# Starlight0798/gymRL

Hardware: AMD Instinct MI355X
Metric: env-steps/sec at N envs/GPU (PPO LunarLander), 1/2/4/8 GPUs + %HBM roofline (higher is better)
Workload: dtype f32; 1 GPU; PPO LunarLander-v3, 4096 vectorised envs per MI355X (BASELINE.json configs[1]); envs_per_gpu=4096, rollout_len=2048, num_epochs=10, num_minibatches=32, minibatch=262144, model=ActorCritic 8-256-256-{256-4,256-1} tanh, 200,965 params, parallelism=single GPU

## Files before the change

### gymrl_amd/csrc/env_lunar.hip

```cpp
#include "env_lunar_device.hpp"

using namespace gymrl;
using namespace gymrl::lunar;

namespace {

__global__ __launch_bounds__(kEnvBlock) void lunar_reset_kernel(void* buf, int n, uint64_t seed,
                                                                int64_t env_id0,
                                                                float* __restrict__ obs_out) {
  __shared__ uint32_t lds_words[kLdsWords * kEnvBlock];
  const Lds lds{lds_words + threadIdx.x};
  LunarState st(buf, n);
  const int role = threadIdx.x & 3;
  const int i = blockIdx.x * kEnvsPerBlock + (threadIdx.x >> 2);
  if (i >= n) return;
  World W;
  float fx, fy, rew, o[8]; bool term;
  init_episode(W, lds, seed, (uint64_t)(env_id0 + i), 0u, fx, fy);
  env_step_once(W, lds, role, 0, seed, (uint64_t)(env_id0 + i), 0u, 0u, fx, fy, o, rew, term);
  world_io(W, lds, role, st.words, n, i, true);
  if (role == 0) {
    st.ep.ep_ret[i] = 0.0; st.ep.ep_len[i] = 0; st.ep.episode[i] = 0u;
    st.spare_episode[i] = kNoSpare;
  }
  store_obs_quad(obs_out, i, role, o);
}

__global__ __launch_bounds__(kEnvBlock) void lunar_refill_kernel(void* buf, int n, uint64_t seed,
                                                                 int64_t env_id0) {
  __shared__ uint32_t lds_words[kLdsWords * kEnvBlock];
  const Lds lds{lds_words + threadIdx.x};
  LunarState st(buf, n);
  const int role = threadIdx.x & 3;
  const int i = blockIdx.x * kEnvsPerBlock + (threadIdx.x >> 2);
  if (i >= n) return;
  const uint32_t want = st.ep.episode[i] + 1u;
  lunar_refill_quad(st, lds, n, i, role, st.spare_episode[i] != want, want, seed, env_id0);
}

__global__ __launch_bounds__(kEnvBlock) void lunar_step_kernel(
    void* buf, int n, uint64_t seed, int64_t env_id0, const int32_t* __restrict__ action,
    float* __restrict__ obs_out, float* __restrict__ term_obs_out, float* __restrict__ rew_out,
    uint8_t* __restrict__ terminated_out, uint8_t* __restrict__ truncated_out,
    uint8_t* __restrict__ done_out, float* __restrict__ ep_ret_out,
    int32_t* __restrict__ ep_len_out, double* __restrict__ ep_stats) {
  __shared__ uint32_t lds_words[kLdsWords * kEnvBlock];
  const Lds lds{lds_words + threadIdx.x};
  const LunarState st(buf, n);
  const int role = threadIdx.x & 3;
  const int i = blockIdx.x * kEnvsPerBlock + (threadIdx.x >> 2);
  const bool valid = i < n;
  const StepOut out{obs_out, term_obs_out, rew_out, terminated_out, truncated_out, done_out, ep_ret_out, ep_len_out, ep_stats};
  float o_next[8];
  lunar_step_quad(st, lds, n, i, role, valid, valid ? action[i] : 0, seed, env_id0, out, o_next);
}

inline int cdiv(int a, int b) { return (a + b - 1) / b; }

}

namespace gymrl {

size_t lunar_state_bytes(int n) { return LunarState(nullptr, n).bytes; }

int lunar_reset(void* state, int n, uint64_t seed, int64_t env_id0, float* obs_out, hipStream_t s) {
  hipLaunchKernelGGL(lunar_reset_kernel, dim3(cdiv(n, kEnvsPerBlock)), dim3(kEnvBlock), 0, s, state, n, seed,
                     env_id0, obs_out);
  GYMRL_CHECK_LAUNCH();
  return 0;
}

int lunar_refill(void* state, int n, uint64_t seed, int64_t env_id0, hipStream_t s) {
  hipLaunchKernelGGL(lunar_refill_kernel, dim3(cdiv(n, kEnvsPerBlock)), dim3(kEnvBlock), 0, s, state, n, seed, env_id0);
  GYMRL_CHECK_LAUNCH();
  return 0;
}

int lunar_step(void* state, int n, uint64_t seed, int64_t env_id0, const int32_t* action,
               float* obs_out, float* term_obs_out, float* rew_out, uint8_t* terminated_out,
               uint8_t* truncated_out, uint8_t* done_out, float* ep_ret_out, int32_t* ep_len_out,
               double* ep_stats, hipStream_t s) {
  hipLaunchKernelGGL(lunar_step_kernel, dim3(cdiv(n, kEnvsPerBlock)), dim3(kEnvBlock), 0, s, state, n, seed,
                     env_id0, action, obs_out, term_obs_out, rew_out, terminated_out, truncated_out,
                     done_out, ep_ret_out, ep_len_out, ep_stats);
  GYMRL_CHECK_LAUNCH();
  return 0;
}

}
```

### gymrl_amd/csrc/env_lunar_device.hpp

```cpp
#pragma once
#include "env_common.hpp"

namespace gymrl {
namespace lunar {


constexpr float kScale = 30.0f;
constexpr float kW = 600.0f / kScale;
constexpr float kH = 400.0f / kScale;
constexpr float kHelipadY = kH / 4.0f;
constexpr float kLegDown = 18.0f / kScale;
constexpr float kLegAway = 20.0f / kScale;
constexpr float kDt = 1.0f / 50.0f;
constexpr int kVelIters = 180, kPosIters = 60, kMaxSteps = 1000;
constexpr float kLinearSlopSqMax = 0x1.a36e30p-16f;
constexpr float kLinearSlop = 0.005f, kAngularSlop = 2.0f / 180.0f * 3.14159265359f;
constexpr float kPolyRadius = 2.0f * kLinearSlop;
constexpr float kMaxLinCorr = 0.2f, kMaxAngCorr = 8.0f / 180.0f * 3.14159265359f;
constexpr float kBaumgarte = 0.2f;
constexpr float kMaxTranslation = 2.0f, kMaxRotation = 0.5f * 3.14159265359f;
constexpr float kTimeToSleep = 0.5f, kLinSleepTol = 0.01f, kAngSleepTol = 2.0f / 180.0f * 3.14159265359f;
constexpr float kMotorTorque = 40.0f;

__device__ constexpr float kInvM[3] = {0.20761245674740486f, 14.0625f, 14.0625f};
__device__ constexpr float kInvI[3] = {1.2757043935679302f, 558.3639705882352f, 558.3639705882352f};
constexpr float kHullLcY = 0.10130718954248369f;
__device__ constexpr float kHullVx[6] = {17.f / 30, 17.f / 30, 14.f / 30, -14.f / 30, -17.f / 30, -17.f / 30};
__device__ constexpr float kHullVy[6] = {-10.f / 30, 0.f, 17.f / 30, 17.f / 30, 0.f, -10.f / 30};
__device__ constexpr float kHullNx[6] = {1.0f, 0.9847835588179369f, 0.0f, -0.9847835588179369f, -1.0f, 0.0f};
__device__ constexpr float kHullNy[6] = {0.0f, 0.17378533390904766f, 1.0f, 0.17378533390904766f, 0.0f, -1.0f};
__device__ constexpr float kLegVx[4] = {-2.f / 30, 2.f / 30, 2.f / 30, -2.f / 30};
__device__ constexpr float kLegVy[4] = {-8.f / 30, -8.f / 30, 8.f / 30, 8.f / 30};
__device__ constexpr float kLegNx[4] = {0.0f, 1.0f, 0.0f, -1.0f};
__device__ constexpr float kLegNy[4] = {-1.0f, 0.0f, 1.0f, 0.0f};

typedef float v2f __attribute__((ext_vector_type(2)));
struct Body { float cx, cy, a, vx, vy, w; };

struct Joint {
  float ix, iy, iz, im;
  int state;
};

struct ContactPt { float lpx, lpy; uint32_t key; float ni, ti; };
struct Manifold {
  int count;
  int faceB;
  float lnx, lny, lpx, lpy;
  ContactPt p[2];
};

constexpr int kMfWords = 16;
constexpr int kVcWords = 17;
constexpr int kLdsWords = 2 * kMfWords + 2 * kVcWords;
constexpr int kQuad = 4;
constexpr int kEnvsPerBlock = kEnvBlock / kQuad;

#ifdef GYMRL_LUNAR_PROF
#define LUNAR_PROF_MARK(var) const unsigned long long var = wall_clock64()
#define LUNAR_PROF_ADD(lds, slot, t0, t1) do { if ((lds).prof && (threadIdx.x & 63) == 0) (lds).prof[slot] += (t1) - (t0); } while (0)
#else
#define LUNAR_PROF_MARK(var)
#define LUNAR_PROF_ADD(lds, slot, t0, t1)
#endif

struct Lds {
  uint32_t* w;
#ifdef GYMRL_LUNAR_PROF
  unsigned long long* prof;
#endif
  uint32_t* park = nullptr;
#ifdef GYMRL_LUNAR_PROF
  unsigned long long* envp = nullptr;
  int envn = 0;
#endif
  __device__ __forceinline__ float& mf(int s, int f) const { return reinterpret_cast<float*>(w)[(s * kMfWords + f) * kEnvBlock]; }
  __device__ __forceinline__ uint32_t& mu(int s, int f) const { return w[(s * kMfWords + f) * kEnvBlock]; }
  __device__ __forceinline__ float& vc(int s, int f) const { return reinterpret_cast<float*>(w)[(2 * kMfWords + s * kVcWords + f) * kEnvBlock]; }
  __device__ __forceinline__ uint32_t& vu(int s, int f) const { return w[(2 * kMfWords + s * kVcWords + f) * kEnvBlock]; }
};

template <int R>
__device__ __forceinline__ float quad_bcast(float x) {
  return __int_as_float(__builtin_amdgcn_update_dpp(0, __float_as_int(x), R * 0x55, 0xF, 0xF, true));
}
template <int CTRL>
__device__ __forceinline__ float quad_perm(float x) {
  return __int_as_float(__builtin_amdgcn_update_dpp(0, __float_as_int(x), CTRL, 0xF, 0xF, true));
}
constexpr int kRot1 = 0xC9;
constexpr int kRot2 = 0xD2;
constexpr int kSwap01 = 0xE1;
template <int R>
__device__ __forceinline__ uint32_t quad_bcast_u(uint32_t x) {
  return (uint32_t)__builtin_amdgcn_update_dpp(0, (int)x, R * 0x55, 0xF, 0xF, true);
}
enum { MF_COUNT = 0, MF_FACEB = 1, MF_LNX = 2, MF_LNY = 3, MF_LPX = 4, MF_LPY = 5, MF_P0 = 6, MF_P1 = 11,
       P_LPX = 0, P_LPY = 1, P_KEY = 2, P_NI = 3, P_TI = 4 };
enum { VC_COUNT = 0, VC_NX = 1, VC_NY = 2, VC_RX0 = 3, VC_RY0 = 4, VC_RX1 = 5, VC_RY1 = 6, VC_NM0 = 7, VC_NM1 = 8,
       VC_TM0 = 9, VC_TM1 = 10, VC_K11 = 11, VC_K12 = 12, VC_K22 = 13, VC_I11 = 14, VC_I12 = 15, VC_I22 = 16 };

struct World {
  Body b[3];
  float sleep[3];
  Joint j[2];
  int edge0;
  uint32_t touching;
  float ty[11];
  uint32_t flags;
  float prev_shaping;
};

__device__ __forceinline__ float cross2(float ax, float ay, float bx, float by) { return ax * by - ay * bx; }
__device__ __forceinline__ float dot2(float ax, float ay, float bx, float by) { return ax * bx + ay * by; }
__device__ __forceinline__ float clampf(float x, float lo, float hi) { return fmaxf(lo, fminf(x, hi)); }

__device__ __forceinline__ float leg_sign(int L) { return L == 0 ? -1.0f : 1.0f; }
__device__ __forceinline__ float joint_lower(int L) { return L == 0 ? 0.4f : -0.9f; }
__device__ __forceinline__ float joint_upper(int L) { return L == 0 ? 0.9f : -0.4f; }

template <int NV>
__device__ __forceinline__ void collide_edge_polygon(Manifold& mf, const float* __restrict__ VX,
                                                     const float* __restrict__ VY,
                                                     const float* __restrict__ NX,
                                                     const float* __restrict__ NY, float px, float py,
                                                     float qs, float qc, float ccx, float ccy,
                                                     float v1x, float v1y, float v2x, float v2y) {
  mf.count = 0;
  float wx[NV], wy[NV], wnx[NV], wny[NV];
#pragma unroll
  for (int i = 0; i < NV; ++i) {
    wx[i] = (qc * VX[i] - qs * VY[i]) + px;
    wy[i] = (qs * VX[i] + qc * VY[i]) + py;
    wnx[i] = qc * NX[i] - qs * NY[i];
    wny[i] = qs * NX[i] + qc * NY[i];
  }
  float ex = v2x - v1x, ey = v2y - v1y;
  const float el = sqrtf(ex * ex + ey * ey);
  const float inv = 1.0f / el;
  ex *= inv; ey *= inv;
  const float n1x = ey, n1y = -ex;
  const float offset1 = dot2(n1x, n1y, ccx - v1x, ccy - v1y);
  const bool front = offset1 >= 0.0f;
  const float Nx = front ? n1x : -n1x, Ny = front ? n1y : -n1y;
  const float radius = 2.0f * kPolyRadius;

  float esep = 3.4e38f;
#pragma unroll
  for (int i = 0; i < NV; ++i) {
    const float s = dot2(Nx, Ny, wx[i] - v1x, wy[i] - v1y);
    if (s < esep) esep = s;
  }
  if (esep > radius) return;
  float psep = -3.4e38f;
  int pidx = -1;
  bool separated = false;
#pragma unroll
  for (int i = 0; i < NV; ++i) {
    const float nx = -wnx[i], ny = -wny[i];
    const float s1 = dot2(nx, ny, wx[i] - v1x, wy[i] - v1y);
    const float s2 = dot2(nx, ny, wx[i] - v2x, wy[i] - v2y);
    const float s = fminf(s1, s2);
    if (!separated) {
      if (s > radius) { separated = true; }
      else if (s > psep) { psep = s; pidx = i; }
    }
  }
  if (separated) return;
  const bool use_edge = (pidx < 0) || !(psep > 0.98f * esep + 0.001f);

  float i0x, i0y, i1x, i1y;
  uint32_t id0, id1;
  float rv1x, rv1y, rv2x, rv2y, rnx, rny;
  int ri1, ri2;
  if (use_edge) {
    int best = 0;
    float bestv = dot2(Nx, Ny, wnx[0], wny[0]);
#pragma unroll
    for (int i = 1; i < NV; ++i) {
      const float v = dot2(Nx, Ny, wnx[i], wny[i]);
      if (v < bestv) { bestv = v; best = i; }
    }
    const int b2 = best + 1 < NV ? best + 1 : 0;
    i0x = wx[0]; i0y = wy[0]; i1x = wx[0]; i1y = wy[0];
#pragma unroll
    for (int i = 0; i < NV; ++i) {
      if (i == best) { i0x = wx[i]; i0y = wy[i]; }
      if (i == b2) { i1x = wx[i]; i1y = wy[i]; }
    }
    id0 = 0u | ((uint32_t)best << 8) | (1u << 16) | (0u << 24);
    id1 = 0u | ((uint32_t)b2 << 8) | (1u << 16) | (0u << 24);
    if (front) { ri1 = 0; ri2 = 1; rv1x = v1x; rv1y = v1y; rv2x = v2x; rv2y = v2y; rnx = n1x; rny = n1y; }
    else { ri1 = 1; ri2 = 0; rv1x = v2x; rv1y = v2y; rv2x = v1x; rv2y = v1y; rnx = -n1x; rny = -n1y; }
  } else {
    i0x = v1x; i0y = v1y; i1x = v2x; i1y = v2y;
    id0 = 0u | ((uint32_t)pidx << 8) | (0u << 16) | (1u << 24);
    id1 = 0u | ((uint32_t)pidx << 8) | (0u << 16) | (1u << 24);
    ri1 = pidx; ri2 = pidx + 1 < NV ? pidx + 1 : 0;
    rv1x = wx[0]; rv1y = wy[0]; rv2x = wx[0]; rv2y = wy[0]; rnx = wnx[0]; rny = wny[0];
#pragma unroll
    for (int i = 0; i < NV; ++i) {
      if (i == ri1) { rv1x = wx[i]; rv1y = wy[i]; rnx = wnx[i]; rny = wny[i]; }
      if (i == ri2) { rv2x = wx[i]; rv2y = wy[i]; }
    }
  }
  const float sn1x = rny, sn1y = -rnx;
  const float so1 = dot2(sn1x, sn1y, rv1x, rv1y);
  const float so2 = dot2(-sn1x, -sn1y, rv2x, rv2y);

  float c0x, c0y, c1x, c1y; uint32_t cid0, cid1; int np = 0;
  {
    const float d0 = dot2(sn1x, sn1y, i0x, i0y) - so1;
    const float d1 = dot2(sn1x, sn1y, i1x, i1y) - so1;
    c0x = c0y = c1x = c1y = 0.0f; cid0 = cid1 = 0u;
    if (d0 <= 0.0f) { c0x = i0x; c0y = i0y; cid0 = id0; np = 1; }
    if (d1 <= 0.0f) { if (np == 0) { c0x = i1x; c0y = i1y; cid0 = id1; } else { c1x = i1x; c1y = i1y; cid1 = id1; } ++np; }
    if (d0 * d1 < 0.0f) {
      const float t = d0 / (d0 - d1);
      const float nxp = i0x + t * (i1x - i0x), nyp = i0y + t * (i1y - i0y);
      const uint32_t nid = (uint32_t)ri1 | (((id0 >> 8) & 0xFFu) << 8) | (0u << 16) | (1u << 24);
      if (np == 0) { c0x = nxp; c0y = nyp; cid0 = nid; } else { c1x = nxp; c1y = nyp; cid1 = nid; }
      ++np;
    }
  }
  if (np < 2) return;
  float e0x, e0y, e1x, e1y; uint32_t eid0, eid1; np = 0;
  {
    const float d0 = dot2(-sn1x, -sn1y, c0x, c0y) - so2;
    const float d1 = dot2(-sn1x, -sn1y, c1x, c1y) - so2;
    e0x = e0y = e1x = e1y = 0.0f; eid0 = eid1 = 0u;
    if (d0 <= 0.0f) { e0x = c0x; e0y = c0y; eid0 = cid0; np = 1; }
    if (d1 <= 0.0f) { if (np == 0) { e0x = c1x; e0y = c1y; eid0 = cid1; } else { e1x = c1x; e1y = c1y; eid1 = cid1; } ++np; }
    if (d0 * d1 < 0.0f) {
      const float t = d0 / (d0 - d1);
      const float nxp = c0x + t * (c1x - c0x), nyp = c0y + t * (c1y - c0y);
      const uint32_t nid = (uint32_t)ri2 | (((cid0 >> 8) & 0xFFu) << 8) | (0u << 16) | (1u << 24);
      if (np == 0) { e0x = nxp; e0y = nyp; eid0 = nid; } else { e1x = nxp; e1y = nyp; eid1 = nid; }
      ++np;
    }
  }
  if (np < 2) return;

  mf.faceB = use_edge ? 0 : 1;
  if (use_edge) { mf.lnx = rnx; mf.lny = rny; mf.lpx = rv1x; mf.lpy = rv1y; }
  else {
    mf.lnx = NX[0]; mf.lny = NY[0]; mf.lpx = VX[0]; mf.lpy = VY[0];
#pragma unroll
    for (int i = 0; i < NV; ++i) if (i == ri1) { mf.lnx = NX[i]; mf.lny = NY[i]; mf.lpx = VX[i]; mf.lpy = VY[i]; }
  }
  int cnt = 0;
#pragma unroll
  for (int k = 0; k < 2; ++k) {
    const float qx = k == 0 ? e0x : e1x, qy = k == 0 ? e0y : e1y;
    const uint32_t qid = k == 0 ? eid0 : eid1;
    const float sep = dot2(rnx, rny, qx - rv1x, qy - rv1y);
    if (sep <= radius) {
      float lx, ly; uint32_t key;
      if (use_edge) {
        const float dx = qx - px, dy = qy - py;
        lx = qc * dx + qs * dy; ly = -qs * dx + qc * dy;
        key = qid;
      } else {
        lx = qx; ly = qy;
        key = ((qid >> 8) & 0xFFu) | ((qid & 0xFFu) << 8) | (((qid >> 24) & 0xFFu) << 16) | (((qid >> 16) & 0xFFu) << 24);
// ... 270 lines not shown
    }
    quad_share_velocity(B, me);
  }

  float jrAx[2], jrAy[2], jrBx[2], jrBy[2];
  float K11[2], K12[2], K13[2], K22[2], K23[2], K33[2], mmass[2];
  {
    float qsA, qcA;
    det_sincosf(B[0].a, &qsA, &qcA);
#pragma unroll
    for (int jj = 0; jj < 2; ++jj) {
      const int L = 1 - jj;
      const int bi = L + 1;
      float qsB, qcB;
      det_sincosf(B[bi].a, &qsB, &qcB);
      const float lax = 0.0f - 0.0f, lay = 0.0f - kHullLcY;
      const float lbx = leg_sign(L) * kLegAway, lby = kLegDown;
      jrAx[L] = qcA * lax - qsA * lay; jrAy[L] = qsA * lax + qcA * lay;
      jrBx[L] = qcB * lbx - qsB * lby; jrBy[L] = qsB * lbx + qcB * lby;
      const float mA = kInvM[0], mB = kInvM[bi], iA = kInvI[0], iB = kInvI[bi];
      K11[L] = mA + mB + jrAy[L] * jrAy[L] * iA + jrBy[L] * jrBy[L] * iB;
      K12[L] = -jrAy[L] * jrAx[L] * iA - jrBy[L] * jrBx[L] * iB;
      K13[L] = -jrAy[L] * iA - jrBy[L] * iB;
      K22[L] = mA + mB + jrAx[L] * jrAx[L] * iA + jrBx[L] * jrBx[L] * iB;
      K23[L] = jrAx[L] * iA + jrBx[L] * iB;
      K33[L] = iA + iB;
      mmass[L] = 1.0f / (iA + iB);
      Joint& J = W.j[L];
      const float ang = B[bi].a - B[0].a;
      if (ang <= joint_lower(L)) { if (J.state != 1) J.iz = 0.0f; J.state = 1; }
      else if (ang >= joint_upper(L)) { if (J.state != 2) J.iz = 0.0f; J.state = 2; }
      else { J.state = 0; J.iz = 0.0f; }
      const float Px = J.ix, Py = J.iy;
      B[0].vx -= mA * Px; B[0].vy -= mA * Py;
      B[0].w -= iA * (cross2(jrAx[L], jrAy[L], Px, Py) + J.im + J.iz);
      B[bi].vx += mB * Px; B[bi].vy += mB * Py;
      B[bi].w += iB * (cross2(jrBx[L], jrBy[L], Px, Py) + J.im + J.iz);
    }
  }

  LUNAR_PROF_MARK(pt2);
  LUNAR_PROF_ADD(lds, 1, pt1, pt2);
  float jpAx[2], jpAy[2], jpBx[2], jpBy[2];
  float c1x[2], c1y[2], c1z[2], det3i[2], det2i[2], lim_sign[2];
  bool at_limit[2];
#pragma unroll
  for (int L = 0; L < 2; ++L) {
    const float a11 = K11[L], a12 = K12[L], a13 = K13[L], a22 = K22[L], a23 = K23[L], a33 = K33[L];
    c1x[L] = a22 * a33 - a23 * a23; c1y[L] = a23 * a13 - a12 * a33; c1z[L] = a12 * a23 - a22 * a13;
    float det = a11 * c1x[L] + a12 * c1y[L] + a13 * c1z[L];
    if (det != 0.0f) det = 1.0f / det;
    det3i[L] = det;
    float d2 = a11 * a22 - a12 * a12;
    if (d2 != 0.0f) d2 = 1.0f / d2;
    det2i[L] = d2;
    jpAx[L] = -jrAy[L]; jpAy[L] = jrAx[L]; jpBx[L] = -jrBy[L]; jpBy[L] = jrBx[L];
    at_limit[L] = W.j[L].state != 0;
    lim_sign[L] = W.j[L].state == 1 ? 1.0f : -1.0f;
  }
  const bool r0 = role == 0, r1 = role == 1, r2 = role == 2;
  auto lane3 = [&](float x, float y, float z) { return r0 ? x : (r1 ? y : (r2 ? z : 0.0f)); };
  float JPA[2], JPB[2], C1[2], P2[2], Q2[2], A2[2], P3[2], Q3[2], A3[2], A3C[2], D2[2], MBv[2], IBz[2];
#pragma unroll
  for (int L = 0; L < 2; ++L) {
    const float a11 = K11[L], a12 = K12[L], a13 = K13[L], a22 = K22[L], a23 = K23[L], a33 = K33[L];
    JPA[L] = lane3(jpAx[L], jpAy[L], 0.0f); JPB[L] = lane3(jpBx[L], jpBy[L], 0.0f);
    C1[L] = lane3(c1x[L], c1y[L], c1z[L]);
    P2[L] = lane3(a23, a33, a13); Q2[L] = lane3(a13, a23, a33); A2[L] = lane3(a13, a11, a12);
    P3[L] = lane3(a23, a12, a22); Q3[L] = lane3(a12, a22, a23); A3[L] = lane3(a12, a13, a11);
    A3C[L] = lane3(a13, a23, 0.0f); D2[L] = lane3(a22, a11, 0.0f);
    MBv[L] = lane3(kInvM[L + 1], kInvM[L + 1], kInvI[L + 1]); IBz[L] = r2 ? kInvI[L + 1] : 0.0f;
  }
  const float MAv = lane3(kInvM[0], kInvM[0], kInvI[0]), IAz = r2 ? kInvI[0] : 0.0f;
  float VA = lane3(B[0].vx, B[0].vy, B[0].w);
  float VB[2] = {lane3(B[1].vx, B[1].vy, B[1].w), lane3(B[2].vx, B[2].vy, B[2].w)};
  float JI[2] = {lane3(W.j[0].ix, W.j[0].iy, W.j[0].iz), lane3(W.j[1].ix, W.j[1].iy, W.j[1].iz)};
  float IM[2] = {W.j[0].im, W.j[1].im};
  const float maxImp = h * kMotorTorque;
#define SB __builtin_amdgcn_sched_barrier(0)
#define USEL(c, a, b) (__builtin_unpredictable(c) ? (a) : (b))
  float zb[2];
  zb[1] = quad_perm<0xAA>(JI[1]) * A3C[1];
  zb[0] = 0.0f;
  float lim_nan[2] = {at_limit[0] ? lim_sign[0] : __builtin_nanf(""), at_limit[1] ? lim_sign[1] : __builtin_nanf("")};
  asm volatile("" : "+v"(lim_nan[0]), "+v"(lim_nan[1]));
  auto joints = [&]() {
#pragma unroll
    for (int jj = 0; jj < 2; ++jj) {
      const int L = 1 - jj;
      const bool lim = at_limit[L];
      float t = VB[L] - VA; SB;
      t = t - 0.3f * leg_sign(L); SB;
      float imp = -mmass[L] * t; SB;
      float nw = IM[L] + imp; SB;
      nw = __builtin_amdgcn_fmed3f(nw, -maxImp, maxImp); SB;
      imp = nw - IM[L]; IM[L] = nw; SB;
      const float mb_ = IBz[L] * imp; SB;
      VB[L] = VB[L] + mb_; SB;
      const float ma_ = IAz * imp; SB;
      VA = VA - ma_; SB;
      const float xb = quad_perm<0xAA>(VB[L]) * JPB[L]; SB;
      float c = VB[L] + xb; SB;
      const float xa = quad_perm<0xAA>(VA) * JPA[L]; SB;
      c = c - VA; SB;
      c = c - xa; SB;
      const float u1 = c * C1[L]; SB;
      const float zc = zb[L] - c; SB;
      const float q2 = quad_perm<kRot1>(c) * Q2[L]; SB;
      const float q3 = quad_perm<kRot2>(c) * Q3[L]; SB;
      const float m2 = c * P2[L] - q2; SB;
      const float m3 = c * P3[L] - q3; SB;
      float s1 = quad_perm<kRot1>(u1) + u1; SB;
      const float u2 = A2[L] * m2; SB;
      const float u3 = A3[L] * m3; SB;
      s1 = quad_perm<kRot2>(u1) + s1; SB;
      const float rr = USEL(lim, zc, -c); SB;
      float s2 = quad_perm<kRot1>(u2) + u2; SB;
      float s3 = quad_perm<kRot1>(u3) + u3; SB;
      const float d2r = D2[L] * rr; SB;
      s2 = quad_perm<kRot2>(u2) + s2; SB;
      s3 = quad_perm<kRot2>(u3) + s3; SB;
      const float r2_ = quad_perm<kSwap01>(rr) * K12[L]; SB;
      float sel = USEL(r1, s2, s3); SB;
      sel = USEL(r0, s1, sel); SB;
      const float nsol = -(det3i[L] * sel); SB;
      const float newJ = JI[L] + nsol; SB;
      const float uu = d2r - r2_; SB;
      const float u = det2i[L] * uu; SB;
      const float rt = quad_perm<0xAA>(newJ) * lim_nan[L]; SB;
      const float altz = USEL(lim, -JI[L], 0.0f); SB;
      const float alt = USEL(r2, altz, u); SB;
      float ip;
      asm("v_cmp_nge_f32 vcc, %1, 0\n\tv_cndmask_b32_e32 %0, %2, %3, vcc" : "=v"(ip) : "v"(rt), "v"(nsol), "v"(alt) : "vcc"); SB;
      JI[L] = JI[L] + ip; SB;
      zb[1 - L] = quad_perm<0xAA>(JI[1 - L]) * A3C[1 - L]; SB;
      const float ay = quad_perm<0x55>(ip) * jrAx[L]; SB;
      const float ax = quad_perm<0x00>(ip) * jrAy[L]; SB;
      const float by = quad_perm<0x55>(ip) * jrBx[L]; SB;
      const float bx = quad_perm<0x00>(ip) * jrBy[L]; SB;
      const float crA = ay - ax; SB;
      const float crB = by - bx; SB;
      const float wA = crA + ip; SB;
      const float wB = crB + ip; SB;
      float tA = USEL(r2, wA, ip); SB;
      float tB = USEL(r2, wB, ip); SB;
      tA = MAv * tA; SB;
      tB = MBv[L] * tB; SB;
      VA = VA - tA; SB;
      VB[L] = VB[L] + tB; SB;
    }
  };
#undef SB
#undef USEL
  auto contacts = [&]() {
    if (any_contact) {
      Body me;
      me.cx = me.cy = me.a = 0.0f;
      me.vx = sel3(mb, quad_bcast<0>(VA), quad_bcast<0>(VB[0]), quad_bcast<0>(VB[1]));
      me.vy = sel3(mb, quad_bcast<1>(VA), quad_bcast<1>(VB[0]), quad_bcast<1>(VB[1]));
      me.w = sel3(mb, quad_bcast<2>(VA), quad_bcast<2>(VB[0]), quad_bcast<2>(VB[1]));
#pragma unroll
      for (int s = 0; s < 2; ++s) {
        const int vcount = vcn[s];
        if (vcount > 0) {
          const float nx = vcf[s][VC_NX - 1], ny = vcf[s][VC_NY - 1], tx = ny, ty = -nx;
          const float rx0 = vcf[s][VC_RX0 - 1], ry0 = vcf[s][VC_RY0 - 1], rx1 = vcf[s][VC_RX1 - 1], ry1 = vcf[s][VC_RY1 - 1];
          float ni0 = vim[s][0], ti0 = vim[s][1], ni1 = vim[s][2], ti1 = vim[s][3];
          {
            const float dvx = me.vx + (-me.w * ry0), dvy = me.vy + (me.w * rx0);
            const float vt = dot2(dvx, dvy, tx, ty);
            float lam = vcf[s][VC_TM0 - 1] * (-vt);
            const float maxF = fr_ * ni0;
            const float nw = clampf(ti0 + lam, -maxF, maxF);
            lam = nw - ti0; ti0 = nw;
            const float Px = lam * tx, Py = lam * ty;
            me.vx += mB_ * Px; me.vy += mB_ * Py;
            me.w += iB_ * cross2(rx0, ry0, Px, Py);
          }
          if (vcount == 2) {
            const float dvx = me.vx + (-me.w * ry1), dvy = me.vy + (me.w * rx1);
            const float vt = dot2(dvx, dvy, tx, ty);
            float lam = vcf[s][VC_TM1 - 1] * (-vt);
            const float maxF = fr_ * ni1;
            const float nw = clampf(ti1 + lam, -maxF, maxF);
            lam = nw - ti1; ti1 = nw;
            const float Px = lam * tx, Py = lam * ty;
            me.vx += mB_ * Px; me.vy += mB_ * Py;
            me.w += iB_ * cross2(rx1, ry1, Px, Py);
          }
          if (vcount == 1) {
            const float dvx = me.vx + (-me.w * ry0), dvy = me.vy + (me.w * rx0);
            const float vn = dot2(dvx, dvy, nx, ny);
            float lam = -vcf[s][VC_NM0 - 1] * vn;
            const float nw = fmaxf(ni0 + lam, 0.0f);
            lam = nw - ni0; ni0 = nw;
            const float Px = lam * nx, Py = lam * ny;
            me.vx += mB_ * Px; me.vy += mB_ * Py;
            me.w += iB_ * cross2(rx0, ry0, Px, Py);
          } else {
            const float k11 = vcf[s][VC_K11 - 1], k12 = vcf[s][VC_K12 - 1], k22 = vcf[s][VC_K22 - 1];
            const float a1 = ni0, a2 = ni1;
            const float dv1x = me.vx + (-me.w * ry0), dv1y = me.vy + (me.w * rx0);
            const float dv2x = me.vx + (-me.w * ry1), dv2y = me.vy + (me.w * rx1);
            float vn1 = dot2(dv1x, dv1y, nx, ny), vn2 = dot2(dv2x, dv2y, nx, ny);
            const float b1 = vn1 - (k11 * a1 + k12 * a2);
            const float b2 = vn2 - (k12 * a1 + k22 * a2);
            float x1 = -(vcf[s][VC_I11 - 1] * b1 + vcf[s][VC_I12 - 1] * b2);
            float x2 = -(vcf[s][VC_I12 - 1] * b1 + vcf[s][VC_I22 - 1] * b2);
            bool ok = (x1 >= 0.0f && x2 >= 0.0f);
            if (!ok) {
              x1 = -vcf[s][VC_NM0 - 1] * b1; x2 = 0.0f;
              vn2 = k12 * x1 + b2;
              ok = (x1 >= 0.0f && vn2 >= 0.0f);
            }
            if (!ok) {
              x1 = 0.0f; x2 = -vcf[s][VC_NM1 - 1] * b2;
              vn1 = k12 * x2 + b1;
              ok = (x2 >= 0.0f && vn1 >= 0.0f);
            }
            if (!ok) {
              x1 = 0.0f; x2 = 0.0f;
              ok = (b1 >= 0.0f && b2 >= 0.0f);
            }
            if (ok) {
              const float d1 = x1 - a1, d2 = x2 - a2;
              const float P1x = d1 * nx, P1y = d1 * ny, P2x = d2 * nx, P2y = d2 * ny;
              me.vx += mB_ * (P1x + P2x); me.vy += mB_ * (P1y + P2y);
              me.w += iB_ * (cross2(rx0, ry0, P1x, P1y) + cross2(rx1, ry1, P2x, P2y));
              ni0 = x1; ni1 = x2;
            }
          }
          vim[s][0] = ni0; vim[s][1] = ti0;
          if (vcount == 2) { vim[s][2] = ni1; vim[s][3] = ti1; }
        }
      }
      VA = lane3(quad_bcast<0>(me.vx), quad_bcast<0>(me.vy), quad_bcast<0>(me.w));
      VB[0] = lane3(quad_bcast<1>(me.vx), quad_bcast<1>(me.vy), quad_bcast<1>(me.w));
      VB[1] = lane3(quad_bcast<2>(me.vx), quad_bcast<2>(me.vy), quad_bcast<2>(me.w));
    }
  };
  if (__builtin_amdgcn_ballot_w64(any_contact) == 0ull) {
#pragma nounroll
    for (int it = 0; it < kVelIters; ++it) joints();
  } else {
#pragma nounroll
    for (int it = 0; it < kVelIters; ++it) { joints(); contacts(); }
  }
  B[0].vx = quad_bcast<0>(VA); B[0].vy = quad_bcast<1>(VA); B[0].w = quad_bcast<2>(VA);
#pragma unroll
  for (int L = 0; L < 2; ++L) {
    B[L + 1].vx = quad_bcast<0>(VB[L]); B[L + 1].vy = quad_bcast<1>(VB[L]); B[L + 1].w = quad_bcast<2>(VB[L]);
    W.j[L].ix = quad_bcast<0>(JI[L]); W.j[L].iy = quad_bcast<1>(JI[L]); W.j[L].iz = quad_bcast<2>(JI[L]);
    W.j[L].im = quad_bcast<2>(IM[L]);
  }
  LUNAR_PROF_MARK(pt3);
  LUNAR_PROF_ADD(lds, 2, pt2, pt3);
#ifdef GYMRL_LUNAR_PROF
  const bool wave_contact = __builtin_amdgcn_ballot_w64(any_contact) != 0ull;
  LUNAR_PROF_ADD(lds, wave_contact ? 6 : 7, pt2, pt3);
#endif
  if (my_contact) {
#pragma unroll
    for (int s = 0; s < 2; ++s) {
      if (vcn[s] > 0) {
        lds.mf(s, MF_P0 + P_NI) = vim[s][0]; lds.mf(s, MF_P0 + P_TI) = vim[s][1];
        if (vcn[s] == 2) { lds.mf(s, MF_P1 + P_NI) = vim[s][2]; lds.mf(s, MF_P1 + P_TI) = vim[s][3]; }
      }
    }
  }

#pragma unroll
  for (int b = 0; b < 3; ++b) {
    float tx = h * B[b].vx, ty = h * B[b].vy;
    if (dot2(tx, ty, tx, ty) > kMaxTranslation * kMaxTranslation) {
      const float ratio = kMaxTranslation / sqrtf(dot2(tx, ty, tx, ty));
      B[b].vx *= ratio; B[b].vy *= ratio;
    }
    const float rot = h * B[b].w;
    if (rot * rot > kMaxRotation * kMaxRotation) {
      const float ratio = kMaxRotation / fabsf(rot);
      B[b].w *= ratio;
    }
    B[b].cx += h * B[b].vx; B[b].cy += h * B[b].vy; B[b].a += h * B[b].w;
  }

  LUNAR_PROF_MARK(pt4);
  LUNAR_PROF_ADD(lds, 3, pt3, pt4);
#ifdef GYMRL_LUNAR_PROF
  int prof_pos_iters = 0;
#endif
  bool position_solved = false;
  float plim_value[2], plim_slop[2], plim_lo[2], plim_hi[2];
#pragma unroll
  for (int L = 0; L < 2; ++L) {
    const bool lower = W.j[L].state == 1;
    plim_value[L] = lower ? joint_lower(L) : joint_upper(L);
    plim_slop[L] = lower ? kAngularSlop : -kAngularSlop;
    plim_lo[L] = lower ? -kMaxAngCorr : 0.0f;
    plim_hi[L] = lower ? 0.0f : kMaxAngCorr;
  }
  int pcnt[2] = {0, 0};
  bool pfaceB[2] = {false, false};
  float plnx[2], plny[2], plpx[2], plpy[2], pqx[2][2], pqy[2][2];
#pragma unroll
  for (int s = 0; s < 2; ++s) {
    plnx[s] = plny[s] = plpx[s] = plpy[s] = 0.0f;
    pqx[s][0] = pqx[s][1] = pqy[s][0] = pqy[s][1] = 0.0f;
    if (my_contact) {
      pcnt[s] = (int)lds.mu(s, MF_COUNT);
      pfaceB[s] = lds.mu(s, MF_FACEB) != 0u;
      plnx[s] = lds.mf(s, MF_LNX); plny[s] = lds.mf(s, MF_LNY);
      plpx[s] = lds.mf(s, MF_LPX); plpy[s] = lds.mf(s, MF_LPY);
#pragma unroll
      for (int k = 0; k < 2; ++k) {
        pqx[s][k] = lds.mf(s, MF_P0 + 5 * k + P_LPX); pqy[s][k] = lds.mf(s, MF_P0 + 5 * k + P_LPY);
      }
    }
  }
#pragma nounroll
  for (int it = 0; it < kPosIters; ++it) {
    float min_sep = 0.0f;
    if (any_contact) {
      Body me = select_body(B, mb);
      float my_min = 0.0f;
#pragma unroll
      for (int s = 0; s < 2; ++s) {
        const int cnt = pcnt[s];
        if (cnt > 0) {
          const bool faceB = pfaceB[s];
          const float lnx = plnx[s], lny = plny[s], lpx = plpx[s], lpy = plpy[s];
#pragma unroll
          for (int k = 0; k < 2; ++k) {
            if (k < cnt) {
              const float qx = pqx[s][k], qy = pqy[s][k];
              float px, py, qs, qc;
              body_xf(me, lcy_, px, py, qs, qc);
              float nx, ny, ptx, pty, sep;
              if (!faceB) {
                nx = lnx; ny = lny;
                const float clx = (qc * qx - qs * qy) + px, cly = (qs * qx + qc * qy) + py;
                sep = dot2(clx - lpx, cly - lpy, nx, ny) - kPolyRadius - kPolyRadius;
                ptx = clx; pty = cly;
              } else {
                nx = qc * lnx - qs * lny; ny = qs * lnx + qc * lny;
                const float ppx = (qc * lpx - qs * lpy) + px, ppy = (qs * lpx + qc * lpy) + py;
                sep = dot2(qx - ppx, qy - ppy, nx, ny) - kPolyRadius - kPolyRadius;
                ptx = qx; pty = qy;
                nx = -nx; ny = -ny;
              }
              const float rx = ptx - me.cx, ry = pty - me.cy;
              my_min = fminf(my_min, sep);
              const float C = clampf(kBaumgarte * (sep + kLinearSlop), -kMaxLinCorr, 0.0f);
              const float rn = cross2(rx, ry, nx, ny);
              const float K = mB_ + iB_ * rn * rn;
              const float imp = K > 0.0f ? -C / K : 0.0f;
              const float Px = imp * nx, Py = imp * ny;
              me.cx += mB_ * Px; me.cy += mB_ * Py;
              me.a += iB_ * cross2(rx, ry, Px, Py);
            }
          }
        }
      }
      quad_share_position(B, me);
      min_sep = fminf(fminf(quad_bcast<0>(my_min), quad_bcast<1>(my_min)), quad_bcast<2>(my_min));
    }
    const bool contacts_ok = min_sep >= -3.0f * kLinearSlop;
    bool joints_ok = true;
#pragma unroll
    for (int jj = 0; jj < 2; ++jj) {
      const int L = 1 - jj;
      const int bi = L + 1;
      const float mA = kInvM[0], mB = kInvM[bi], iA = kInvI[0], iB = kInvI[bi];
      const bool lim = at_limit[L];
      const float Cang = (B[bi].a - B[0].a) - plim_value[L];
      const float angErr = lim ? -(lim_sign[L] * Cang) : 0.0f;
      const float Cc = clampf(Cang + plim_slop[L], plim_lo[L], plim_hi[L]);
      const float limImp = lim ? -mmass[L] * Cc : 0.0f;
      B[0].a -= iA * limImp; B[bi].a += iB * limImp;
      float qsA, qcA, qsB, qcB;
      {
        float sn, cs;
        det_sincosf((role & 1) ? B[bi].a : B[0].a, &sn, &cs);
        qsA = quad_bcast<0>(sn); qcA = quad_bcast<0>(cs);
        qsB = quad_bcast<1>(sn); qcB = quad_bcast<1>(cs);
      }
      const float lax = 0.0f, lay = 0.0f - kHullLcY;
      const float lbx = leg_sign(L) * kLegAway, lby = kLegDown;
      const float rAx = qcA * lax - qsA * lay, rAy = qsA * lax + qcA * lay;
      const float rBx = qcB * lbx - qsB * lby, rBy = qsB * lbx + qcB * lby;
      const float Cx = B[bi].cx + rBx - B[0].cx - rAx, Cy = B[bi].cy + rBy - B[0].cy - rAy;
      const float posErr2 = Cx * Cx + Cy * Cy;
      const float k11 = mA + mB + iA * rAy * rAy + iB * rBy * rBy;
      const float k12 = -iA * rAx * rAy - iB * rBx * rBy;
      const float k22 = mA + mB + iA * rAx * rAx + iB * rBx * rBx;
      float det = k11 * k22 - k12 * k12;
      if (det != 0.0f) det = 1.0f / det;
      const float impx = -(det * (k22 * Cx - k12 * Cy)), impy = -(det * (k11 * Cy - k12 * Cx));
      B[0].cx -= mA * impx; B[0].cy -= mA * impy;
      B[0].a -= iA * cross2(rAx, rAy, impx, impy);
// ... 357 lines not shown
```

Before: 7.237 million env-steps/s.

## Specialize contact velocity sweep by wave contact shape and use DPP select asm

The contact velocity solver loop is split into three template variants chosen per wave by ballot: general two-point manifolds, one-point with a second slot, and one-point single-slot. This drops the 2x2 block solver and second-slot branches from the 180-iteration inner loop when no lane in the wave needs them. The quad broadcast/select of body velocities is rewritten as inline DPP v_cndmask asm with precomputed role masks to cut instruction count. An env var forces the general path, at the cost of more code size and hand-written asm that depends on the quad role layout.

```diff
diff --git a/gymrl_amd/csrc/env_lunar.hip b/gymrl_amd/csrc/env_lunar.hip
--- a/gymrl_amd/csrc/env_lunar.hip
+++ b/gymrl_amd/csrc/env_lunar.hip
@@ -1,3 +1,5 @@
+#include <cstdlib>
+
 #include "env_lunar_device.hpp"
 
 using namespace gymrl;
@@ -43,9 +45,10 @@
     float* __restrict__ obs_out, float* __restrict__ term_obs_out, float* __restrict__ rew_out,
     uint8_t* __restrict__ terminated_out, uint8_t* __restrict__ truncated_out,
     uint8_t* __restrict__ done_out, float* __restrict__ ep_ret_out,
-    int32_t* __restrict__ ep_len_out, double* __restrict__ ep_stats) {
+    int32_t* __restrict__ ep_len_out, double* __restrict__ ep_stats, int general_sweep) {
   __shared__ uint32_t lds_words[kLdsWords * kEnvBlock];
-  const Lds lds{lds_words + threadIdx.x};
+  Lds lds{lds_words + threadIdx.x};
+  lds.general_sweep = general_sweep != 0;
   const LunarState st(buf, n);
   const int role = threadIdx.x & 3;
   const int i = blockIdx.x * kEnvsPerBlock + (threadIdx.x >> 2);
@@ -80,9 +83,11 @@
                float* obs_out, float* term_obs_out, float* rew_out, uint8_t* terminated_out,
                uint8_t* truncated_out, uint8_t* done_out, float* ep_ret_out, int32_t* ep_len_out,
                double* ep_stats, hipStream_t s) {
+  const char* gs = getenv("GYMRL_LUNAR_GENERAL_SWEEP");
+  const int general_sweep = gs && gs[0] == '1';
   hipLaunchKernelGGL(lunar_step_kernel, dim3(cdiv(n, kEnvsPerBlock)), dim3(kEnvBlock), 0, s, state, n, seed,
                      env_id0, action, obs_out, term_obs_out, rew_out, terminated_out, truncated_out,
-                     done_out, ep_ret_out, ep_len_out, ep_stats);
+                     done_out, ep_ret_out, ep_len_out, ep_stats, general_sweep);
   GYMRL_CHECK_LAUNCH();
   return 0;
 }
diff --git a/gymrl_amd/csrc/env_lunar_device.hpp b/gymrl_amd/csrc/env_lunar_device.hpp
--- a/gymrl_amd/csrc/env_lunar_device.hpp
+++ b/gymrl_amd/csrc/env_lunar_device.hpp
@@ -74,6 +74,7 @@
   unsigned long long* envp = nullptr;
   int envn = 0;
 #endif
+  bool general_sweep = false;
   __device__ __forceinline__ float& mf(int s, int f) const { return reinterpret_cast<float*>(w)[(s * kMfWords + f) * kEnvBlock]; }
   __device__ __forceinline__ uint32_t& mu(int s, int f) const { return w[(s * kMfWords + f) * kEnvBlock]; }
   __device__ __forceinline__ float& vc(int s, int f) const { return reinterpret_cast<float*>(w)[(2 * kMfWords + s * kVcWords + f) * kEnvBlock]; }
@@ -110,6 +111,8 @@
   uint32_t flags;
   float prev_shaping;
 };
+
+template <bool B> struct SweepFlag { static constexpr bool value = B; };
 
 __device__ __forceinline__ float cross2(float ax, float ay, float bx, float by) { return ax * by - ay * bx; }
 __device__ __forceinline__ float dot2(float ax, float ay, float bx, float by) { return ax * bx + ay * by; }
@@ -686,15 +689,26 @@
   };
 #undef SB
 #undef USEL
-  auto contacts = [&]() {
+  unsigned long long role_not1 = 0xDDDDDDDDDDDDDDDDull, role_not2 = 0xBBBBBBBBBBBBBBBBull, role_12 = 0x6666666666666666ull;
+  asm volatile("" : "+s"(role_not1), "+s"(role_not2), "+s"(role_12));
+#define QSEL3(d, s, R) "v_cndmask_b32_dpp " d ", " s ", " d ", vcc quad_perm:[" R "," R "," R "," R "] row_mask:0xf bank_mask:0xf bound_ctrl:1\n\t"
+#define QMOV3(d, s, R) "v_mov_b32_dpp " d ", " s " quad_perm:[" R "," R "," R "," R "] row_mask:0xf bank_mask:0xf bound_ctrl:1\n\t"
+  auto contacts = [&](auto two_, auto slot1_) {
+    constexpr bool TWO = decltype(two_)::value, SLOT1 = decltype(slot1_)::value;
+    const unsigned long long m_not1 = role_not1, m_not2 = role_not2, m_12 = role_12;
     if (any_contact) {
       Body me;
       me.cx = me.cy = me.a = 0.0f;
-      me.vx = sel3(mb, quad_bcast<0>(VA), quad_bcast<0>(VB[0]), quad_bcast<0>(VB[1]));
-      me.vy = sel3(mb, quad_bcast<1>(VA), quad_bcast<1>(VB[0]), quad_bcast<1>(VB[1]));
-      me.w = sel3(mb, quad_bcast<2>(VA), quad_bcast<2>(VB[0]), quad_bcast<2>(VB[1]));
-#pragma unroll
-      for (int s = 0; s < 2; ++s) {
+      asm(QMOV3("%0", "%5", "0") QMOV3("%1", "%5", "1") QMOV3("%2", "%5", "2")
+          "s_mov_b64 vcc, %6\n\t"
+          QSEL3("%0", "%4", "0") QSEL3("%1", "%4", "1") QSEL3("%2", "%4", "2")
+          "s_mov_b64 vcc, %7\n\t"
+          QSEL3("%0", "%3", "0") QSEL3("%1", "%3", "1") QSEL3("%2", "%3", "2")
+          : "=&v"(me.vx), "=&v"(me.vy), "=&v"(me.w)
+          : "v"(VA), "v"(VB[0]), "v"(VB[1]), "s"(m_not1), "s"(m_12)
+          : "vcc");
+#pragma unroll
+      for (int s = 0; s < (SLOT1 ? 2 : 1); ++s) {
         const int vcount = vcn[s];
         if (vcount > 0) {
           const float nx = vcf[s][VC_NX - 1], ny = vcf[s][VC_NY - 1], tx = ny, ty = -nx;
@@ -711,7 +725,7 @@
             me.vx += mB_ * Px; me.vy += mB_ * Py;
             me.w += iB_ * cross2(rx0, ry0, Px, Py);
           }
-          if (vcount == 2) {
+          if (TWO && vcount == 2) {
             const float dvx = me.vx + (-me.w * ry1), dvy = me.vy + (me.w * rx1);
             const float vt = dot2(dvx, dvy, tx, ty);
             float lam = vcf[s][VC_TM1 - 1] * (-vt);
@@ -722,7 +736,7 @@
             me.vx += mB_ * Px; me.vy += mB_ * Py;
             me.w += iB_ * cross2(rx1, ry1, Px, Py);
           }
-          if (vcount == 1) {
+          if (!TWO || vcount == 1) {
             const float dvx = me.vx + (-me.w * ry0), dvy = me.vy + (me.w * rx0);
             const float vn = dot2(dvx, dvy, nx, ny);
             float lam = -vcf[s][VC_NM0 - 1] * vn;
@@ -765,20 +779,35 @@
             }
           }
           vim[s][0] = ni0; vim[s][1] = ti0;
-          if (vcount == 2) { vim[s][2] = ni1; vim[s][3] = ti1; }
+          if (TWO && vcount == 2) { vim[s][2] = ni1; vim[s][3] = ti1; }
         }
       }
-      VA = lane3(quad_bcast<0>(me.vx), quad_bcast<0>(me.vy), quad_bcast<0>(me.w));
-      VB[0] = lane3(quad_bcast<1>(me.vx), quad_bcast<1>(me.vy), quad_bcast<1>(me.w));
-      VB[1] = lane3(quad_bcast<2>(me.vx), quad_bcast<2>(me.vy), quad_bcast<2>(me.w));
+      asm("s_mov_b64 vcc, %6\n\t"
+          QMOV3("%0", "%3", "0") QMOV3("%1", "%3", "1") QMOV3("%2", "%3", "2")
+          QSEL3("%0", "%4", "0") QSEL3("%1", "%4", "1") QSEL3("%2", "%4", "2")
+          "s_mov_b64 vcc, %7\n\t"
+          QSEL3("%0", "%5", "0") QSEL3("%1", "%5", "1") QSEL3("%2", "%5", "2")
+          : "=&v"(VA), "=&v"(VB[0]), "=&v"(VB[1])
+          : "v"(me.vx), "v"(me.vy), "v"(me.w), "s"(m_not1), "s"(m_not2)
+          : "vcc");
     }
   };
+#undef QSEL3
+#undef QMOV3
+  const bool wave_two = __builtin_amdgcn_ballot_w64(vcn[0] == 2 || vcn[1] == 2) != 0ull || lds.general_sweep;
+  const bool wave_slot1 = __builtin_amdgcn_ballot_w64(vcn[1] > 0) != 0ull;
   if (__builtin_amdgcn_ballot_w64(any_contact) == 0ull) {
 #pragma nounroll
     for (int it = 0; it < kVelIters; ++it) joints();
+  } else if (wave_two) {
+#pragma nounroll
+    for (int it = 0; it < kVelIters; ++it) { joints(); contacts(SweepFlag<true>{}, SweepFlag<true>{}); }
+  } else if (wave_slot1) {
+#pragma nounroll
+    for (int it = 0; it < kVelIters; ++it) { joints(); contacts(SweepFlag<false>{}, SweepFlag<true>{}); }
   } else {
 #pragma nounroll
-    for (int it = 0; it < kVelIters; ++it) { joints(); contacts(); }
+    for (int it = 0; it < kVelIters; ++it) { joints(); contacts(SweepFlag<false>{}, SweepFlag<false>{}); }
   }
   B[0].vx = quad_bcast<0>(VA); B[0].vy = quad_bcast<1>(VA); B[0].w = quad_bcast<2>(VA);
 #pragma unroll
```

After: 7.362 million env-steps/s, median of 6. +1.7%, better.
